# Kolkir/feature-point-cnn

Hardware: AMD Instinct MI355X
Metric: frames/sec (VGA 640x480) SuperPoint fwd+NMS+descriptors (higher is better)
Workload: dtype f32

## Files before the change

feature-point-cnn_amd/csrc/wblock36p_mfma.h:

```cpp
#pragma once
#include "wblock36_mfma.h"

namespace fpc {

template <int TYT_, int TXT_, bool DUST_ = false, bool CONV_ = false>
struct W36PCfg {
  static constexpr int TYT = TYT_, TXT = TXT_;
  static constexpr bool DUST = DUST_, CONV = CONV_;
  static_assert(TYT * TXT == 16 && (TYT == 4 || TYT == 2 || (CONV && !DUST && TYT == 8)), "16 Winograd tiles per workgroup tile: 4 x 4 or 2 x 8 (conv-only: or 8 x 2)");
  static constexpr int NT = 512, NTH = 256, NPOS = 36, KC = 16, N = 64;
  static constexpr int TH = 4 * TYT, TW = 4 * TXT, HH = TH + 2, HW = TW + 2, NHALO = HH * HW;
  static constexpr int HROW = 20;
  static constexpr int HIT = (NHALO * 5 + NTH - 1) / NTH;
  static constexpr int HALO_FLOATS = HIT * NTH * 4;
  static constexpr int V_FLOATS = NPOS * 16 * 16;
  static constexpr int OFF_V0 = 0, OFF_H1 = V_FLOATS, OFF_H0 = OFF_H1 + HALO_FLOATS, OFF_V1 = OFF_H0 + HALO_FLOATS;
  static constexpr int RH = N + 8;
  static constexpr int PX = TH * TW;
  static constexpr int T_FLOATS = PX * RH;
  static constexpr int BASE_FLOATS = (OFF_V1 + V_FLOATS) > (OFF_H0 + T_FLOATS) ? (OFF_V1 + V_FLOATS) : (OFF_H0 + T_FLOATS);
  static constexpr int HIT64 = (NHALO + NTH - 1) / NTH;
  static constexpr int D_HEAD = BASE_FLOATS, D_COL = D_HEAD + 64, D_UIN = D_HEAD + 448, D_V64 = D_UIN + 2304, D_M64 = D_V64 + 576, D_H64 = D_M64 + 576;
  static constexpr int LDS_FLOATS = DUST ? D_H64 + HIT64 * NTH * 4 : BASE_FLOATS;
  static constexpr int LDS_BYTES = LDS_FLOATS * 4;
  static_assert(LDS_BYTES <= 160 * 1024, "LDS");
  static constexpr int STEPS = 9;
  static constexpr int WPAD = W36Cfg<1, 4, 4>::WPAD, WPAD2 = W36Cfg<1, 4, 4>::WPAD2;
  static_assert(WPAD >= 36, "a wave prefetches up to one chunk past its stream's end");
};

template <int TYT, int TXT, int RING, bool DUST, bool CONV = false>
__device__ __forceinline__ void wblock36p_body(const WBlockArgs& a) {
  using C = W36PCfg<TYT, TXT, DUST, CONV>;
  constexpr int TH = C::TH, TW = C::TW, HW = C::HW, HH = C::HH, HROW = C::HROW, HIT = C::HIT, NTH = C::NTH;
  constexpr int N = C::N, RH = C::RH, STEPS = C::STEPS, PX = C::PX;
  static_assert(STEPS % RING == 0 && RING >= 2, "ring slots must line up across chunks");
  extern __shared__ __attribute__((aligned(16))) float lds[];
  f32x4* const lds4 = reinterpret_cast<f32x4*>(lds);
  constexpr int TL4 = C::OFF_H0 / 4;

  const int tid = threadIdx.x, lane = tid & 63;
  const unsigned lane16 = (unsigned)lane * 16u;
  const int wave = __builtin_amdgcn_readfirstlane(tid >> 6);
  const int grp = wave & 3;
  const int hs = wave >> 2;
  const int tiles = a.tiles_x * a.tiles_y;
  const int nchunk = a.nchunk;
  const float4* const w1h = a.w1 + (size_t)blockIdx.y * (a.ysplit_floats / 4);
  const float* const b1h = a.b1 + (size_t)blockIdx.y * a.ysplit_floats;

  const bool xcd_order = a.xcd_order && (gridDim.x & 7) == 0;
  const int wg_step = xcd_order ? (int)(gridDim.x >> 3) : (int)gridDim.x;
  const int xchunk = (a.total + 7) >> 3;
  const int wg_first = xcd_order ? (int)(blockIdx.x & 7) * xchunk + (int)(blockIdx.x >> 3) : (int)blockIdx.x;
  const int wg_end = xcd_order ? min(a.total, ((int)(blockIdx.x & 7) + 1) * xchunk) : a.total;
  if (wg_first >= wg_end) return;

  const __amdgpu_buffer_rsrc_t xrsrc = __builtin_amdgcn_make_buffer_rsrc(const_cast<float*>(a.x), 0, (int)a.x_bytes, 0x00020000);
  struct TilePos { int b, ty, tx, live; };
  auto tile_pos = [&](int wg) {
    TilePos q;
    q.live = wg < wg_end;
    const int wgc = q.live ? wg : wg_first;
    const int bl = wgc / tiles;
    const int t = wgc - bl * tiles;
    q.b = a.frame0 + bl;
    q.ty = t / a.tiles_x;
    q.tx = t - q.ty * a.tiles_x;
    return q;
  };
  auto halo_base = [&](const TilePos& q) {
    return __builtin_amdgcn_readfirstlane(((q.b * a.H + q.ty * TH) * a.W + q.tx * TW) * a.csx * 4);
  };
  constexpr bool KEEP_HYX = !DUST;
  auto slot_hyx = [&](int tl, int i) {
    const int e = tl + i * NTH;
    const int pix = (e * 13108) >> 16, c4 = e - pix * 5;
    const int hy = HW == 18 ? (pix * 3641) >> 16 : HW == 34 ? (pix * 1928) >> 16 : (pix * 6554) >> 16;
    static_assert(HW == 18 || HW == 34 || HW == 10, "a division constant per halo width");
    const int hx = pix - hy * HW;
    const bool slot_ok = (hy < HH) & (c4 < 4);
    return slot_ok ? (hy << 16) | (c4 << 8) | hx : 0x7fff0000;
  };
  int okoff[HIT];
  [[maybe_unused]] int hyx[KEEP_HYX ? HIT : 1];
  if (hs == 1) {
    const int tl = tid & (NTH - 1);
#pragma unroll
    for (int i = 0; i < HIT; ++i) {
      if constexpr (KEEP_HYX) hyx[i] = slot_hyx(tl, i);
      okoff[i] = W36_MARKER;
    }
  }
  [[maybe_unused]] int okoff64[C::HIT64];
  auto slot_hyx64 = [&](int tl, int i) {
    const int pix = tl + i * NTH;
    const int hy = HW == 18 ? (pix * 3641) >> 16 : HW == 34 ? (pix * 1928) >> 16 : (pix * 6554) >> 16;
    const int hx = pix - hy * HW;
    return (hy < HH && a.dust_in) ? (hy << 16) | hx : 0x7fff0000;
  };
  if constexpr (DUST) {
    if (hs == 1) {
#pragma unroll
      for (int i = 0; i < C::HIT64; ++i) okoff64[i] = W36_MARKER;
    }
  }
  auto halo_tile = [&](const TilePos& q) {
    const int iy0 = q.ty * TH - 1, ix0 = q.tx * TW - 1;
    const int hlim = q.live ? a.H : 0;
    int tlq = tid & (NTH - 1);
    asm volatile("" : "+v"(tlq));
#pragma unroll
    for (int i = 0; i < HIT; ++i) {
      int hv = KEEP_HYX ? hyx[KEEP_HYX ? i : 0] : slot_hyx(tlq, i);
      asm volatile("" : "+v"(hv));
      const int hy = hv >> 16, hx = hv & 0xff, c4 = (hv >> 8) & 0xff;
      const bool ok = ((unsigned)(iy0 + hy) < (unsigned)hlim) & ((unsigned)(ix0 + hx) < (unsigned)a.W);
      okoff[i] = ok ? (((hy - 1) * a.W + (hx - 1)) * a.csx + c4 * 4) * 4 : W36_MARKER;
    }
    if constexpr (DUST) {
#pragma unroll
      for (int i = 0; i < C::HIT64; ++i) {
        int hv = slot_hyx64(tlq, i);
        asm volatile("" : "+v"(hv));
        const int hy = hv >> 16, hx = hv & 0xffff;
        const bool ok = ((unsigned)(iy0 + hy) < (unsigned)hlim) & ((unsigned)(ix0 + hx) < (unsigned)a.W);
        okoff64[i] = ok ? (((hy - 1) * a.W + (hx - 1)) * a.csx + 64) * 4 : W36_MARKER;
      }
    }
  };
  auto load_halo64 = [&](int base) {
    if constexpr (DUST) {
#pragma unroll
      for (int i = 0; i < C::HIT64; ++i) {
        int voff;
        asm("v_add_i32 %0, %1, %2 clamp" : "=v"(voff) : "v"(okoff64[i]), "s"(base));
        __builtin_amdgcn_raw_ptr_buffer_load_lds(xrsrc, (__attribute__((address_space(3))) void*)(lds + C::D_H64 + (i * NTH + grp * 64) * 4), 16, voff, 0, 0, 0);
      }
    }
  };
  auto load_halo = [&](int base, int hoff_f) {
#pragma unroll
    for (int i = 0; i < HIT; ++i) {
      int voff;
      asm("v_add_i32 %0, %1, %2 clamp" : "=v"(voff) : "v"(okoff[i]), "s"(base));
      __builtin_amdgcn_raw_ptr_buffer_load_lds(xrsrc, (__attribute__((address_space(3))) void*)(lds + hoff_f + (i * NTH + grp * 64) * 4), 16, voff, 0, 0, 0);
    }
  };
  const int tq = tid & (NTH - 1);
  const int wt_t = tq >> 4, ch_t = tq & 15;
  const int m_t = ((wt_t & 7) >> 1) * 4 + (wt_t >> 3) * 2 + (wt_t & 1);
  const int trd = ((4 * (wt_t / TXT)) * HW + 4 * (wt_t % TXT)) * HROW + ch_t;
  const int twr = m_t * 16 + ((((ch_t >> 2) ^ (2 * ((m_t >> 3) & 1))) << 2) | (ch_t & 3));
  typedef float f32x2 __attribute__((ext_vector_type(2)));
  f32x2 tp[6][3];
  auto t_read = [&](int rd, int i, int j) { tp[i][j >> 1][j & 1] = lds[rd + (i * HW + j) * HROW]; };
  auto bt6 = [&](f32x2& x0, f32x2& x1, f32x2& x2, f32x2& x3, f32x2& x4, f32x2& x5) {
    const f32x2 k4 = {4.f, 4.f}, km4 = {-4.f, -4.f}, k5 = {-5.f, -5.f}, k2 = {2.f, 2.f}, km2 = {-2.f, -2.f};
    const f32x2 p = __builtin_elementwise_fma(km4, x2, x4), q = __builtin_elementwise_fma(km4, x1, x3);
    const f32x2 r = x4 - x2, s = x3 - x1;
    const f32x2 y0 = __builtin_elementwise_fma(k4, x0, __builtin_elementwise_fma(k5, x2, x4));
    const f32x2 y5 = __builtin_elementwise_fma(k4, x1, __builtin_elementwise_fma(k5, x3, x5));
    x0 = y0;
    x1 = p + q;
    x2 = p - q;
    x3 = __builtin_elementwise_fma(k2, s, r);
    x4 = __builtin_elementwise_fma(km2, s, r);
    x5 = y5;
  };
  auto t_burst = [&]() {
#pragma unroll
    for (int jj = 0; jj < 3; ++jj) bt6(tp[0][jj], tp[1][jj], tp[2][jj], tp[3][jj], tp[4][jj], tp[5][jj]);
#pragma unroll
    for (int ii = 0; ii < 3; ++ii)
#pragma unroll
      for (int jj = 0; jj < 3; ++jj) {
        const f32x2 ra = tp[2 * ii][jj], rb = tp[2 * ii + 1][jj];
        tp[2 * ii][jj] = __builtin_shufflevector(ra, rb, 0, 2);
        tp[2 * ii + 1][jj] = __builtin_shufflevector(ra, rb, 1, 3);
      }
#pragma unroll
    for (int ii = 0; ii < 3; ++ii) bt6(tp[2 * ii][0], tp[2 * ii + 1][0], tp[2 * ii][1], tp[2 * ii + 1][1], tp[2 * ii][2], tp[2 * ii + 1][2]);
  };
  auto t_write = [&](int wr, int i, int j) { lds[wr + (i * 6 + j) * 256] = tp[2 * (i >> 1) + (j & 1)][j >> 1][i & 1]; };

  const int aoff4 = (lane & 15) * 4 + ((lane >> 4) ^ (2 * ((lane & 15) >> 3))) + hs * 18 * 64;
  const unsigned gstride = ((unsigned)nchunk * 36u + (unsigned)C::WPAD) * 1024u;
  const __amdgpu_buffer_rsrc_t wrsrc = __builtin_amdgcn_make_buffer_rsrc(const_cast<float4*>(w1h), 0, (int)(4u * gstride), 0x00020000);
  const unsigned wlane = (unsigned)grp * gstride + (unsigned)hs * (18u * 1024u) + lane16;
  struct BF { f32x4 v[2]; };
  auto ldb = [&](int cc, int s) {
    BF r;
#pragma unroll
    for (int q = 0; q < 2; ++q)
      r.v[q] = __builtin_bit_cast(f32x4, __builtin_amdgcn_raw_buffer_load_b128(wrsrc, (int)wlane, cc * (36 * 1024) + (2 * s + q) * 1024, 0));
    return r;
  };

  [[maybe_unused]] int d_va = 0, d_ua = 0;
  [[maybe_unused]] const __amdgpu_buffer_rsrc_t drsrc =
      DUST ? __builtin_amdgcn_make_buffer_rsrc(const_cast<float*>(a.dust + W36Dust::UOUT), 0, nchunk * 36 * 16 * 4, 0x00020000) : xrsrc;
  [[maybe_unused]] f32x4 du[6];
  [[maybe_unused]] float dacc[9];
  if constexpr (DUST) {
    d_va = grp * 64 + lane;
    d_ua = grp * 64 + 16 * ((lane & 3) ^ (2 * (lane >> 5)));
    for (int i = tid; i < 448 / 4; i += C::NT) lds4[C::D_HEAD / 4 + i] = reinterpret_cast<const f32x4*>(a.dust)[i];
    for (int i = tid; i < 2304 / 4; i += C::NT) lds4[C::D_UIN / 4 + i] = reinterpret_cast<const f32x4*>(a.dust + W36Dust::UIN)[i];
  }

  TilePos pos_cur = tile_pos(wg_first);
  int base_cur = halo_base(pos_cur);
  if (hs == 1) {
    halo_tile(pos_cur);
    load_halo64(base_cur);
    load_halo(base_cur, C::OFF_H0);
    load_halo(base_cur + 64, C::OFF_H1);
    asm volatile("s_waitcnt vmcnt(%0)" ::"n"(HIT) : "memory");
  }
  FPC_LDS_BARRIER();
  if (hs == 0) {
#pragma unroll
    for (int i = 0; i < 6; ++i)
#pragma unroll
      for (int j = 0; j < 6; ++j) t_read(trd + C::OFF_H0, i, j);
    t_burst();
#pragma unroll
    for (int i = 0; i < 6; ++i)
#pragma unroll
      for (int j = 0; j < 6; ++j) t_write(twr + C::OFF_V0, i, j);
  }
  FPC_LDS_BARRIER();

  constexpr int C4 = N / 4, EIT = PX * C4 / C::NT, PPI = C::NT / C4;
  constexpr int RPI = PPI / TW > 0 ? PPI / TW : 1;
  const __amdgpu_buffer_rsrc_t orsrc = __builtin_amdgcn_make_buffer_rsrc(a.out + blockIdx.y * N, 0, W36_MARKER, 0x00020000);
  const int g2s = __builtin_amdgcn_readfirstlane(((a.k8_h + a.k8_x) / 2 + C::WPAD2) * 64);
  const __amdgpu_buffer_rsrc_t w2rsrc = __builtin_amdgcn_make_buffer_rsrc(const_cast<float4*>(a.w2), 0, a.conv_only ? 0 : 4 * g2s * 16, 0x00020000);
  const unsigned w2lane = (unsigned)(grp * g2s) * 16u + lane16;

  const int wg_stamp = wg_first + 2 * wg_step < wg_end ? wg_first + 2 * wg_step : wg_first;
  for (int wg = wg_first; wg < wg_end; wg += wg_step) {
    const int b = pos_cur.b, ty = pos_cur.ty, tx = pos_cur.tx;
    const TilePos pos_next = tile_pos(wg + wg_step);
    const int base_next = halo_base(pos_next);
    if (wg == wg_stamp) { FPC_STAMP(0) FPC_RSTAMP(6) }

    f32x4 acc[18];
    {
      float zf = 0.f;
      asm volatile("" : "+v"(zf));
#pragma unroll
      for (int p = 0; p < 18; ++p) acc[p] = f32x4{zf, zf, zf, zf};
    }
    if constexpr (DUST) {
      float zf = 0.f;
      asm volatile("" : "+v"(zf));
#pragma unroll
      for (int i = 0; i < 9; ++i) dacc[i] = zf;
    }
    BF bq[RING];
#pragma unroll
    for (int i = 0; i < RING - 1; ++i) bq[i] = ldb(0, i);

    auto chunk_body = [&](auto ROLE, auto PAR, const int c) {
      constexpr int role = decltype(ROLE)::value, par = decltype(PAR)::value;
      constexpr int VB_OFF = par ? C::OFF_V1 : C::OFF_V0, VN_OFF = par ? C::OFF_V0 : C::OFF_V1;
      constexpr int HS_OFF = par ? C::OFF_H1 : C::OFF_H0;
      constexpr int HN_OFF = par ? C::OFF_H0 : C::OFF_H1;
      const int c3 = c + 2;
      const bool nxt = c3 >= nchunk;
      const int l_base = (nxt ? base_next : base_cur) + (nxt ? c3 - nchunk : c3) * 64;
      int ao = aoff4 + VB_OFF / 4, trd_c = trd + HN_OFF, twr_c = twr + VN_OFF;
      asm volatile("" : "+v"(ao), "+v"(trd_c), "+v"(twr_c));
      [[maybe_unused]] int dva = d_va + VB_OFF / 4;
      [[maybe_unused]] f32x4 dv[3];
      if constexpr (DUST) asm volatile("" : "+v"(dva));
      f32x4 ac[2][2];
#pragma unroll
      for (int q = 0; q < 2; ++q) ac[0][q] = lds4[ao + q * 64];
      fpc_static_for<STEPS>([&](auto S) __attribute__((always_inline)) {
        constexpr int s = decltype(S)::value;
        {
          constexpr int t = s + RING - 1;
          if constexpr (t < STEPS) bq[t % RING] = ldb(c, t);
          else bq[t % RING] = ldb(c + 1, t - STEPS);
        }
        if (s + 1 < STEPS) {
#pragma unroll
          for (int q = 0; q < 2; ++q) ac[(s + 1) & 1][q] = lds4[ao + ((s + 1) * 2 + q) * 64];
        }
        constexpr int SPS = 4;
#pragma unroll
        for (int u = 0; u < SPS; ++u) {
          const int slot = s * SPS + u;
          if constexpr (role == 1) {
            if (slot == 1) {
              if (c3 == nchunk) halo_tile(pos_next);
              load_halo(l_base, HS_OFF);
            }
            if constexpr (DUST) {
              auto dread = [&](int i0) {
#pragma unroll
                for (int k = 0; k < 3; ++k) dv[k] = lds4[dva + (i0 + k) * 256];
              };
              auto dfma = [&](int i0) {
#pragma unroll
                for (int k = 0; k < 3; ++k)
#pragma unroll
                  for (int e = 0; e < 4; ++e) dacc[i0 + k] = __builtin_fmaf(dv[k][e], du[(i0 / 3 % 2) * 3 + k][e], dacc[i0 + k]);
              };
              auto dload = [&](int i0) {
#pragma unroll
                for (int k = 0; k < 3; ++k)
                  du[(i0 / 3 % 2) * 3 + k] = __builtin_bit_cast(f32x4, __builtin_amdgcn_raw_buffer_load_b128(drsrc, d_ua + (i0 + k) * 256, c * (36 * 16 * 4), 0));
              };
              if (slot == 3) dload(0);
              else if (slot == 11) dread(0);
              else if (slot == 13) { dfma(0); dload(3); }
              else if (slot == 21) dread(3);
              else if (slot == 23) { dfma(3); dload(6); }
              else if (slot == 31) dread(6);
              else if (slot == 33) dfma(6);
            }
          } else {
            if (slot >= 2 && slot < 14) {
#pragma unroll
              for (int k = 0; k < 3; ++k) { const int e = (slot - 2) * 3 + k; t_read(trd_c, e / 6, e % 6); }
            } else if (slot == 14) {
              t_burst();
            } else if (slot >= 15 && slot < 33) {
#pragma unroll
              for (int k = 0; k < 2; ++k) { const int e = (slot - 15) * 2 + k; t_write(twr_c, e / 6, e % 6); }
            }
          }
        }
        __builtin_amdgcn_sched_barrier(0);
        fpc_mfma_step<false, false>(acc[2 * s], acc[2 * s + 1], ac[s & 1][0], ac[s & 1][1], bq[s % RING].v[0], bq[s % RING].v[1]);
        __builtin_amdgcn_sched_barrier(0);
      });
      asm volatile("s_waitcnt vmcnt(%0)" ::"n"(2 * (STEPS - 1)) : "memory");
      FPC_LDS_BARRIER();
    };
    __builtin_amdgcn_s_waitcnt(0x0F70);
    if (hs == 0) {
      int c = 0;
      do {
        chunk_body(std::integral_constant<int, 0>{}, std::integral_constant<int, 0>{}, c);
        chunk_body(std::integral_constant<int, 0>{}, std::integral_constant<int, 1>{}, c + 1);
        c += 2;
      } while (c < nchunk);
    } else {
      int c = 0;
      do {
        chunk_body(std::integral_constant<int, 1>{}, std::integral_constant<int, 0>{}, c);
        chunk_body(std::integral_constant<int, 1>{}, std::integral_constant<int, 1>{}, c + 1);
        c += 2;
      } while (c < nchunk);
    }
    if (wg == wg_stamp) { FPC_STAMP(1) }
    asm volatile("s_nop 15\n\ts_nop 7" ::: "memory");

    int tid_t = tid;
    asm volatile("" : "+v"(tid_t));
    const int lane_t = tid_t & 63, n16 = lane_t & 15, kq = lane_t >> 4;
    const bool proj = a.k8_x > 0;
    if constexpr (DUST) {
      if (a.dust_in) {
        if (tid_t < 16) {
          const int rd = C::D_H64 + ((4 * (tid_t / TXT)) * HW + 4 * (tid_t % TXT)) * 4;
#pragma unroll
          for (int i = 0; i < 6; ++i)
#pragma unroll
            for (int j = 0; j < 6; ++j) tp[i][j >> 1][j & 1] = lds[rd + (i * HW + j) * 4];
          t_burst();
          const int mrow = ((tid_t & 7) >> 1) * 4 + (tid_t >> 3) * 2 + (tid_t & 1);
#pragma unroll
          for (int i = 0; i < 6; ++i)
#pragma unroll
            for (int j = 0; j < 6; ++j) lds[C::D_V64 + (i * 6 + j) * 16 + mrow] = tp[2 * (i >> 1) + (j & 1)][j >> 1][i & 1];
        }
        FPC_LDS_BARRIER();
        {
          const int va = C::D_V64 + hs * 18 * 16 + (lane_t & 15), ub = C::D_UIN + grp * 576 + hs * 18 * 16 + (lane_t & 15);
          float av[18], bv[18];
#pragma unroll
          for (int p = 0; p < 18; ++p) {
            av[p] = lds[va + p * 16];
            bv[p] = lds[ub + p * 16];
          }
          __builtin_amdgcn_sched_barrier(0);
#pragma unroll
          for (int p = 0; p < 18; ++p) {
            const float x = lane_t < 16 ? av[p] : 0.f;
            acc[p] = __builtin_amdgcn_mfma_f32_16x16x4f32(x, bv[p], acc[p], 0, 0, 0);
          }
        }
      }
      if (hs == 1) {
        const int m_d = lane_t >> 2;
#pragma unroll
        for (int i = 0; i < 9; ++i) {
          float v = dacc[i];
          v += __shfl_xor(v, 1);
          v += __shfl_xor(v, 2);
          const int pos = grp + 4 * i;
          if (a.dust_in) v = __builtin_fmaf(lds[C::D_V64 + pos * 16 + m_d], lds[C::D_HEAD + W36Dust::UIN64 + pos], v);
          if ((lane_t & 3) == 0) lds[C::D_M64 + pos * 16 + m_d] = v;
        }
      }
      FPC_LDS_BARRIER();
      if (hs == 1) load_halo64(base_next);
    }

    int hw_base[4];
#pragma unroll
    for (int r = 0; r < 4; ++r) {
      const int T = 8 * (r >> 1) + 2 * kq + (r & 1);
      hw_base[r] = C::OFF_H0 + ((4 * (T / TXT)) * TW + 4 * (T % TXT)) * RH + 16 * grp + n16;
    }
    auto out_transform = [&](auto ROLE) __attribute__((always_inline)) {
      constexpr int role = decltype(ROLE)::value;
      auto partial = [&](int rp, f32x2 (&yv)[4][4]) {
        f32x2 tt[4][6];
#pragma unroll
        for (int j = 0; j < 6; ++j) {
          auto pr = [&](int pos) { return f32x2{acc[pos][2 * rp], acc[pos][2 * rp + 1]}; };
          const f32x2 ma = pr(0 * 6 + j), mb = pr(1 * 6 + j), mc = pr(2 * 6 + j);
          if constexpr (role == 0) {
            const f32x2 s12 = mb + mc, d12 = mb - mc;
            tt[0][j] = ma + s12;
            tt[1][j] = d12;
            tt[2][j] = s12;
            tt[3][j] = d12;
          } else {
            const f32x2 s34 = ma + mb, d34 = ma - mb;
            tt[0][j] = s34;
            tt[1][j] = f32x2{2.f, 2.f} * d34;
            tt[2][j] = f32x2{4.f, 4.f} * s34;
            tt[3][j] = __builtin_elementwise_fma(f32x2{8.f, 8.f}, d34, mc);
          }
        }
#pragma unroll
        for (int i = 0; i < 4; ++i) {
          const f32x2 m0 = tt[i][0], m1 = tt[i][1], m2 = tt[i][2], m3 = tt[i][3], m4 = tt[i][4], m5 = tt[i][5];
          const f32x2 s12 = m1 + m2, d12 = m1 - m2, s34 = m3 + m4, d34 = m3 - m4;
          yv[i][0] = m0 + s12 + s34;
          yv[i][1] = __builtin_elementwise_fma(f32x2{2.f, 2.f}, d34, d12);
          yv[i][2] = __builtin_elementwise_fma(f32x2{4.f, 4.f}, s34, s12);
          yv[i][3] = __builtin_elementwise_fma(f32x2{8.f, 8.f}, d34, d12) + m5;
        }
      };
      {
        f32x2 yv[4][4];
        partial(1 - role, yv);
#pragma unroll
        for (int e = 0; e < 2; ++e)
#pragma unroll
          for (int i = 0; i < 4; ++i) lds4[TL4 + (e * 4 + i) * C::NT + tid_t] = f32x4{yv[i][0][e], yv[i][1][e], yv[i][2][e], yv[i][3][e]};
      }
      FPC_LDS_BARRIER();
      {
        f32x4 other[2][4];
#pragma unroll
        for (int e = 0; e < 2; ++e)
#pragma unroll
          for (int i = 0; i < 4; ++i) other[e][i] = lds4[TL4 + (e * 4 + i) * C::NT + (tid_t ^ NTH)];
        f32x2 yv[4][4];
        partial(role, yv);
        const float bias1 = b1h[16 * grp + n16];
        float hv[2][16];
#pragma unroll
        for (int i = 0; i < 4; ++i)
#pragma unroll
          for (int jj = 0; jj < 4; ++jj)
#pragma unroll
            for (int e = 0; e < 2; ++e) {
              const float v = (yv[i][jj][e] + other[e][i][jj]) + bias1;
              hv[e][i * 4 + jj] = v > 0.f ? v : 0.f;
            }
        FPC_LDS_BARRIER();
#pragma unroll
        for (int e = 0; e < 2; ++e)
#pragma unroll
          for (int i = 0; i < 4; ++i)
#pragma unroll
            for (int jj = 0; jj < 4; ++jj) lds[hw_base[2 * role + e] + (i * TW + jj) * RH] = hv[e][i * 4 + jj];
        if constexpr (DUST && role == 0) {
          if (tid_t < 16) {
            float mm[36];
#pragma unroll
            for (int p = 0; p < 36; ++p) mm[p] = lds[C::D_M64 + p * 16 + tid_t];
            const float bias64 = lds[C::D_HEAD + W36Dust::B1];
            float tt[4][6];
#pragma unroll
            for (int j = 0; j < 6; ++j) {
              const float m0 = mm[0 * 6 + j], m1 = mm[1 * 6 + j], m2 = mm[2 * 6 + j], m3 = mm[3 * 6 + j], m4 = mm[4 * 6 + j], m5 = mm[5 * 6 + j];
              const float s12 = m1 + m2, d12 = m1 - m2, s34 = m3 + m4, d34 = m3 - m4;
              tt[0][j] = m0 + s12 + s34;
              tt[1][j] = __builtin_fmaf(2.f, d34, d12);
              tt[2][j] = __builtin_fmaf(4.f, s34, s12);
              tt[3][j] = __builtin_fmaf(8.f, d34, d12) + m5;
            }
            const int T = 8 * ((tid_t >> 1) & 1) + 2 * (tid_t >> 2) + (tid_t & 1);
            const int hb = C::OFF_H0 + ((4 * (T / TXT)) * TW + 4 * (T % TXT)) * RH + 64;
#pragma unroll
            for (int i = 0; i < 4; ++i) {
              const float m0 = tt[i][0], m1 = tt[i][1], m2 = tt[i][2], m3 = tt[i][3], m4 = tt[i][4], m5 = tt[i][5];
              const float s12 = m1 + m2, d12 = m1 - m2, s34 = m3 + m4, d34 = m3 - m4;
              float yv64[4];
              yv64[0] = m0 + s12 + s34 + bias64;
              yv64[1] = __builtin_fmaf(2.f, d34, d12) + bias64;
              yv64[2] = __builtin_fmaf(4.f, s34, s12) + bias64;
              yv64[3] = __builtin_fmaf(8.f, d34, d12) + m5 + bias64;
#pragma unroll
              for (int jj = 0; jj < 4; ++jj) lds[hb + (i * TW + jj) * RH] = yv64[jj] > 0.f ? yv64[jj] : 0.f;
            }
          }
        }
      }
      FPC_LDS_BARRIER();
    };
    if (hs == 0) out_transform(std::integral_constant<int, 0>{});
    else out_transform(std::integral_constant<int, 1>{});
    if (wg == wg_stamp) { FPC_STAMP(2) }

    const int y0 = ty * TH, x0 = tx * TW;
    const int rows_valid = min(TH, a.H - y0);
    const int xbase = __builtin_amdgcn_readfirstlane(((b * a.H + y0) * a.W + x0) * a.csx * 4);
    const int obase = __builtin_amdgcn_readfirstlane(((b * a.H + y0) * a.W + x0) * a.cso * 4);
    const int m0 = tid_t / C4, c4t = tid_t - m0 * C4;
    const int rsub = __builtin_amdgcn_readfirstlane(m0 / TW), pcol = m0 % TW;
    const int ocol = (x0 + pcol < a.W) ? (pcol * a.cso + c4t * 4) * 4 : W36_MARKER;
    int erd = TL4 + m0 * (RH / 4) + c4t;
    asm volatile("" : "+v"(erd));
    auto store_out = [&]() {
#pragma unroll
      for (int i = 0; i < EIT; ++i) {
        const int prow = i * RPI + rsub;
        if (prow < rows_valid) {
          f32x4 v = lds4[erd + i * PPI * (RH / 4)];
          if (!CONV && !a.conv_only) {
            v.x = v.x > 0.f ? v.x : 0.f;
            v.y = v.y > 0.f ? v.y : 0.f;
            v.z = v.z > 0.f ? v.z : 0.f;
            v.w = v.w > 0.f ? v.w : 0.f;
          }
          int voff;
          const int so = obase + prow * a.W * a.cso * 4;
          asm("v_add_i32 %0, %1, %2 clamp" : "=v"(voff) : "v"(ocol), "s"(so));
          __builtin_amdgcn_raw_buffer_store_b128(__builtin_bit_cast(__attribute__((__vector_size__(4 * sizeof(unsigned)))) unsigned, v), orsrc, voff, 0, 0);
        }
      }
    };

    if (CONV || a.conv_only) {
      store_out();
      FPC_LDS_BARRIER();
    } else if constexpr (!CONV) {
      f32x4 acc2[8];
      const int pb = hs;
      [[maybe_unused]] float dpart[8];
      [[maybe_unused]] float dw2r = 0.f;
      [[maybe_unused]] float dhv[8][4];
      [[maybe_unused]] const int dq = lane_t & 15, dpxl = lane_t >> 4;
      [[maybe_unused]] float dx64 = 0.f;
      if constexpr (DUST) {
        if (!proj) {
          const int px = 32 * wave + 4 * (dq >> 1) + dpxl;
          dx64 = __builtin_bit_cast(float, __builtin_amdgcn_raw_buffer_load_b32(xrsrc, (((px / TW) * a.W + px % TW) * a.csx + 64) * 4, xbase, 0));
        }
        const f32x4 wq = lds4[C::D_COL / 4 + dq];
        const float w64 = dq == 0 ? lds[C::D_COL + 64] : 0.f;
#pragma unroll
        for (int it = 0; it < 8; ++it) {
          const int px = 32 * wave + 4 * it + dpxl;
          const f32x4 hq = lds4[TL4 + px * (RH / 4) + dq];
          const float h64 = lds[C::OFF_H0 + px * RH + 64];
          float v = h64 * w64;
#pragma unroll
          for (int e = 0; e < 4; ++e) v = __builtin_fmaf(hq[e], wq[e], v);
          dpart[it] = v;
        }
        dw2r = lds[C::D_HEAD + W36Dust::W2ROW + 16 * grp + n16];
#pragma unroll
        for (int mb = 0; mb < 8; ++mb)
#pragma unroll
          for (int r = 0; r < 4; ++r) dhv[mb][r] = lds[C::OFF_H0 + (128 * pb + 16 * mb + 4 * kq + r) * RH + 64];
      }
      auto ldb2 = [&](int s) {
        return __builtin_bit_cast(f32x4, __builtin_amdgcn_raw_buffer_load_b128(w2rsrc, (int)w2lane, s * 1024, 0));
      };
      constexpr int KH = N / 16;
      auto gemm_over = [&](int ksteps, int s_first) {
        int ar = TL4 + (128 * pb + n16) * (RH / 4) + kq;
        asm volatile("" : "+v"(ar));
        f32x4 cb[4];
#pragma unroll
        for (int i = 0; i < 3; ++i) cb[i] = ldb2(s_first + i);
        f32x4 af[2][2];
#pragma unroll
        for (int q = 0; q < 2; ++q) af[0][q] = lds4[ar + q * 16 * (RH / 4)];
        for (int g = 0; g < ksteps; g += 4) {
#pragma unroll
          for (int u = 0; u < 4; ++u) {
            cb[(u + 3) & 3] = ldb2(s_first + g + u + 3);
            fpc_static_for<4>([&](auto B_) __attribute__((always_inline)) {
              constexpr int blk = decltype(B_)::value;
              if (blk + 1 < 4) {
#pragma unroll
                for (int q = 0; q < 2; ++q) af[(blk + 1) & 1][q] = lds4[ar + (g + u) * 4 + ((blk + 1) * 2 + q) * 16 * (RH / 4)];
              } else {
#pragma unroll
                for (int q = 0; q < 2; ++q) af[(blk + 1) & 1][q] = lds4[ar + (g + u + 1) * 4 + q * 16 * (RH / 4)];
              }
              __builtin_amdgcn_sched_barrier(0);
              fpc_mfma_step<false, false>(acc2[2 * blk], acc2[2 * blk + 1], af[blk & 1][0], af[blk & 1][1], cb[u], cb[u]);
              __builtin_amdgcn_sched_barrier(0);
            });
          }
        }
      };
      if (proj) {
        constexpr int XIT = PX * 16 / C::NT;
        f32x4 xst[XIT];
        auto load_x = [&](int pass) {
          const int kx4 = min(16, a.k8_x * 2 - pass * 16);
          const int px0 = tid_t >> 4;
          const int xp = (((px0 / TW) * a.W + px0 % TW) * a.csx + ((tid_t & 15) < kx4 ? pass * 64 + (tid_t & 15) * 4 : 0)) * 4;
#pragma unroll
          for (int i = 0; i < XIT; ++i) {
            const int so = xbase + i * RPI * a.W * a.csx * 4;
            xst[i] = __builtin_bit_cast(f32x4, __builtin_amdgcn_raw_buffer_load_b128(xrsrc, xp + so, 0, 0));
          }
        };
        load_x(0);
        {
          float zf = 0.f;
          asm volatile("" : "+v"(zf));
#pragma unroll
          for (int mb = 0; mb < 8; ++mb) acc2[mb] = f32x4{zf, zf, zf, zf};
          if constexpr (DUST) {
#pragma unroll
            for (int mb = 0; mb < 8; ++mb)
#pragma unroll
              for (int r = 0; r < 4; ++r) acc2[mb][r] = dhv[mb][r] * dw2r;
          }
        }
        gemm_over(KH, 0);
        if (wg == wg_stamp) { FPC_STAMP(3) }
        const int npass = (a.k8_x + 7) >> 3;
        for (int pass = 0; pass < npass; ++pass) {
          FPC_LDS_BARRIER();
          {
            int xw = TL4 + (tid_t >> 4) * (RH / 4) + (tid_t & 15);
            asm volatile("" : "+v"(xw));
#pragma unroll
            for (int i = 0; i < XIT; ++i) lds4[xw + i * 32 * (RH / 4)] = xst[i];
          }
          FPC_LDS_BARRIER();
          if (pass + 1 < npass) load_x(pass + 1);
          if constexpr (DUST) {
            const f32x4 wa = lds4[C::D_COL / 4 + 20 + pass * 16 + dq];
#pragma unroll
            for (int it = 0; it < 8; ++it) {
              const int px = 32 * wave + 4 * it + dpxl;
              const f32x4 xa = lds4[TL4 + px * (RH / 4) + dq];
              float v = dpart[it];
#pragma unroll
              for (int e = 0; e < 4; ++e) v = __builtin_fmaf(xa[e], wa[e], v);
              dpart[it] = v;
            }
          }
          const int steps = min(4, a.k8_x / 2 - pass * 4);
          gemm_over(steps, KH + pass * 4);
        }
      } else {
        int xl = (4 * kq * a.csx + 16 * grp + n16) * 4;
        asm volatile("" : "+v"(xl));
#pragma unroll
        for (int mb = 0; mb < 8; ++mb)
#pragma unroll
          for (int r = 0; r < 4; ++r) {
            constexpr int BPR = TW / 16;
            const int mbg = 8 * pb + mb;
            const int so = xbase + ((mbg / BPR) * a.W + (mbg % BPR) * 16 + r) * a.csx * 4;
            acc2[mb][r] = __builtin_bit_cast(float, __builtin_amdgcn_raw_buffer_load_b32(xrsrc, xl, so, 0));
          }
        if constexpr (DUST) {
#pragma unroll
          for (int mb = 0; mb < 8; ++mb)
#pragma unroll
            for (int r = 0; r < 4; ++r) acc2[mb][r] = __builtin_fmaf(dhv[mb][r], dw2r, acc2[mb][r]);
        }
        gemm_over(KH, 0);
        if (wg == wg_stamp) { FPC_STAMP(3) }
      }

      if (wg == wg_stamp) { FPC_STAMP(4) }
      asm volatile("s_nop 15\n\ts_nop 7" ::: "memory");
      FPC_LDS_BARRIER();
      {
        int ew = C::OFF_H0 + (128 * pb + 4 * kq) * RH + 16 * grp + n16;
        asm volatile("" : "+v"(ew));
        const float bias = a.b2[16 * grp + n16];
#pragma unroll
        for (int mb = 0; mb < 8; ++mb)
#pragma unroll
          for (int r = 0; r < 4; ++r) lds[ew + (16 * mb + r) * RH] = acc2[mb][r] + bias;
      }
      FPC_LDS_BARRIER();
      store_out();
      if constexpr (DUST) {
        const bool b3 = (dq & 8) != 0, b2 = (dq & 4) != 0, b1 = (dq & 2) != 0;
        float r1[4], r2[2];
#pragma unroll
        for (int k = 0; k < 4; ++k) r1[k] = (b3 ? dpart[4 + k] : dpart[k]) + __shfl_xor(b3 ? dpart[k] : dpart[4 + k], 8);
#pragma unroll
        for (int k = 0; k < 2; ++k) r2[k] = (b2 ? r1[2 + k] : r1[k]) + __shfl_xor(b2 ? r1[k] : r1[2 + k], 4);
        float tot = (b1 ? r2[1] : r2[0]) + __shfl_xor(b1 ? r2[0] : r2[1], 2);
        tot += __shfl_xor(tot, 1);
        const int dpx = 32 * wave + 4 * (dq >> 1) + dpxl, dhf = dq & 1, drow = dpx / TW, dcol = dpx % TW;
        tot += dx64 + lds[C::D_HEAD + W36Dust::B2];
        tot = tot > 0.f ? tot : 0.f;
        const bool ok = (drow < rows_valid) & (x0 + dcol < a.W);
        const int doff = ok ? ((drow * a.W + dcol) * a.cso + 64 + 4 * dhf) * 4 : W36_MARKER;
        int voff;
        asm("v_add_i32 %0, %1, %2 clamp" : "=v"(voff) : "v"(doff), "s"(obase));
        const f32x4 v = {dhf ? 0.f : tot, 0.f, 0.f, 0.f};
        __builtin_amdgcn_raw_buffer_store_b128(__builtin_bit_cast(__attribute__((__vector_size__(4 * sizeof(unsigned)))) unsigned, v), orsrc, voff, 0, 0);
      }
      if (wg == wg_stamp) { FPC_STAMP(5) FPC_RSTAMP(7) }
      FPC_LDS_BARRIER();
    }
    pos_cur = pos_next;
    base_cur = base_next;
  }
}

template <int TYT, int TXT, int RING = 3>
__global__ __launch_bounds__(512, 1) void wblock36p_kernel(const WBlockArgs a) {
  wblock36p_body<TYT, TXT, RING, false>(a);
}

template <int TYT, int TXT, int RING = 3>
__global__ __launch_bounds__(512, 1) void wconv36p_kernel(const WBlockArgs a) {
  wblock36p_body<TYT, TXT, RING, false, true>(a);
}

template <int TYT, int TXT, int RING = 3>
__global__ __launch_bounds__(512, 1) void wblock36p_dust_kernel(const WBlockArgs a) {
  wblock36p_body<TYT, TXT, RING, true>(a);
}

}
```

Baseline: 12380.

## Restructure dust-channel halo setup, 64th-channel output transform, and identity-load addressing

Splits the 64th-channel halo offset computation into its own lambda that runs per tile. It also keeps the precomputed halo coordinates in the dust variant too. The output transform for channel 64 is spread across four wave groups, one output row each, instead of running on 16 threads of role 0. Inline-asm v_fmac replaces the builtin fma in the dust accumulation, and the identity-add load addresses are built incrementally from scalar strides. The aim is to cut VALU and scalar address arithmetic and to balance the serial dust tail, at the cost of more live registers and redundant LDS reads of m-values per row.

```diff
diff --git a/feature-point-cnn_amd/csrc/wblock36p_mfma.h b/feature-point-cnn_amd/csrc/wblock36p_mfma.h
--- a/feature-point-cnn_amd/csrc/wblock36p_mfma.h
+++ b/feature-point-cnn_amd/csrc/wblock36p_mfma.h
@@ -29,6 +29,10 @@
   static_assert(WPAD >= 36, "a wave prefetches up to one chunk past its stream's end");
 };
 
+__device__ __forceinline__ void w36p_fmac(float& d, float x, float y) {
+  asm volatile("v_fmac_f32 %0, %1, %2" : "+v"(d) : "v"(x), "v"(y));
+}
+
 template <int TYT, int TXT, int RING, bool DUST, bool CONV = false>
 __device__ __forceinline__ void wblock36p_body(const WBlockArgs& a) {
   using C = W36PCfg<TYT, TXT, DUST, CONV>;
@@ -72,7 +76,6 @@
   auto halo_base = [&](const TilePos& q) {
     return __builtin_amdgcn_readfirstlane(((q.b * a.H + q.ty * TH) * a.W + q.tx * TW) * a.csx * 4);
   };
-  constexpr bool KEEP_HYX = !DUST;
   auto slot_hyx = [&](int tl, int i) {
     const int e = tl + i * NTH;
     const int pix = (e * 13108) >> 16, c4 = e - pix * 5;
@@ -83,12 +86,12 @@
     return slot_ok ? (hy << 16) | (c4 << 8) | hx : 0x7fff0000;
   };
   int okoff[HIT];
-  [[maybe_unused]] int hyx[KEEP_HYX ? HIT : 1];
+  int hyx[HIT];
   if (hs == 1) {
     const int tl = tid & (NTH - 1);
 #pragma unroll
     for (int i = 0; i < HIT; ++i) {
-      if constexpr (KEEP_HYX) hyx[i] = slot_hyx(tl, i);
+      hyx[i] = slot_hyx(tl, i);
       okoff[i] = W36_MARKER;
     }
   }
@@ -108,17 +111,21 @@
   auto halo_tile = [&](const TilePos& q) {
     const int iy0 = q.ty * TH - 1, ix0 = q.tx * TW - 1;
     const int hlim = q.live ? a.H : 0;
-    int tlq = tid & (NTH - 1);
-    asm volatile("" : "+v"(tlq));
 #pragma unroll
     for (int i = 0; i < HIT; ++i) {
-      int hv = KEEP_HYX ? hyx[KEEP_HYX ? i : 0] : slot_hyx(tlq, i);
+      int hv = hyx[i];
       asm volatile("" : "+v"(hv));
       const int hy = hv >> 16, hx = hv & 0xff, c4 = (hv >> 8) & 0xff;
       const bool ok = ((unsigned)(iy0 + hy) < (unsigned)hlim) & ((unsigned)(ix0 + hx) < (unsigned)a.W);
       okoff[i] = ok ? (((hy - 1) * a.W + (hx - 1)) * a.csx + c4 * 4) * 4 : W36_MARKER;
     }
+  };
+  auto halo_tile64 = [&](const TilePos& q) {
     if constexpr (DUST) {
+      const int iy0 = q.ty * TH - 1, ix0 = q.tx * TW - 1;
+      const int hlim = q.live ? a.H : 0;
+      int tlq = tid & (NTH - 1);
+      asm volatile("" : "+v"(tlq));
 #pragma unroll
       for (int i = 0; i < C::HIT64; ++i) {
         int hv = slot_hyx64(tlq, i);
@@ -203,7 +210,7 @@
   [[maybe_unused]] f32x4 du[6];
   [[maybe_unused]] float dacc[9];
   if constexpr (DUST) {
-    d_va = grp * 64 + lane;
+    d_va = grp * 64 + lane - aoff4;
     d_ua = grp * 64 + 16 * ((lane & 3) ^ (2 * (lane >> 5)));
     for (int i = tid; i < 448 / 4; i += C::NT) lds4[C::D_HEAD / 4 + i] = reinterpret_cast<const f32x4*>(a.dust)[i];
     for (int i = tid; i < 2304 / 4; i += C::NT) lds4[C::D_UIN / 4 + i] = reinterpret_cast<const f32x4*>(a.dust + W36Dust::UIN)[i];
@@ -213,6 +220,7 @@
   int base_cur = halo_base(pos_cur);
   if (hs == 1) {
     halo_tile(pos_cur);
+    halo_tile64(pos_cur);
     load_halo64(base_cur);
     load_halo(base_cur, C::OFF_H0);
     load_halo(base_cur + 64, C::OFF_H1);
@@ -273,9 +281,8 @@
       const int l_base = (nxt ? base_next : base_cur) + (nxt ? c3 - nchunk : c3) * 64;
       int ao = aoff4 + VB_OFF / 4, trd_c = trd + HN_OFF, twr_c = twr + VN_OFF;
       asm volatile("" : "+v"(ao), "+v"(trd_c), "+v"(twr_c));
-      [[maybe_unused]] int dva = d_va + VB_OFF / 4;
+      [[maybe_unused]] const int dva = ao + d_va;
       [[maybe_unused]] f32x4 dv[3];
-      if constexpr (DUST) asm volatile("" : "+v"(dva));
       f32x4 ac[2][2];
 #pragma unroll
       for (int q = 0; q < 2; ++q) ac[0][q] = lds4[ao + q * 64];
@@ -308,7 +315,8 @@
 #pragma unroll
                 for (int k = 0; k < 3; ++k)
 #pragma unroll
-                  for (int e = 0; e < 4; ++e) dacc[i0 + k] = __builtin_fmaf(dv[k][e], du[(i0 / 3 % 2) * 3 + k][e], dacc[i0 + k]);
+                  for (int e = 0; e < 4; ++e)
+                    w36p_fmac(dacc[i0 + k], dv[k][e], du[(i0 / 3 % 2) * 3 + k][e]);
               };
               auto dload = [&](int i0) {
 #pragma unroll
@@ -410,7 +418,10 @@
         }
       }
       FPC_LDS_BARRIER();
-      if (hs == 1) load_halo64(base_next);
+      if (hs == 1) {
+        halo_tile64(pos_next);
+        load_halo64(base_next);
+      }
     }
 
     int hw_base[4];
@@ -486,36 +497,41 @@
           for (int i = 0; i < 4; ++i)
 #pragma unroll
             for (int jj = 0; jj < 4; ++jj) lds[hw_base[2 * role + e] + (i * TW + jj) * RH] = hv[e][i * 4 + jj];
-        if constexpr (DUST && role == 0) {
-          if (tid_t < 16) {
-            float mm[36];
-#pragma unroll
-            for (int p = 0; p < 36; ++p) mm[p] = lds[C::D_M64 + p * 16 + tid_t];
+        if constexpr (DUST && role == 1) {
+          auto y64_row = [&](auto I_) __attribute__((always_inline)) {
+            constexpr int i = decltype(I_)::value;
+            int ma = C::D_M64 + lane_t;
+            asm volatile("" : "+v"(ma));
+            float tt[6];
+#pragma unroll
+            for (int j = 0; j < 6; ++j) {
+              auto mrd = [&](int r) { return lds[ma + (r * 6 + j) * 16]; };
+              const float m1 = mrd(1), m2 = mrd(2), m3 = mrd(3), m4 = mrd(4);
+              const float s12 = m1 + m2, d12 = m1 - m2, s34 = m3 + m4, d34 = m3 - m4;
+              if constexpr (i == 0) tt[j] = mrd(0) + s12 + s34;
+              else if constexpr (i == 1) tt[j] = __builtin_fmaf(2.f, d34, d12);
+              else if constexpr (i == 2) tt[j] = __builtin_fmaf(4.f, s34, s12);
+              else tt[j] = __builtin_fmaf(8.f, d34, d12) + mrd(5);
+            }
             const float bias64 = lds[C::D_HEAD + W36Dust::B1];
-            float tt[4][6];
-#pragma unroll
-            for (int j = 0; j < 6; ++j) {
-              const float m0 = mm[0 * 6 + j], m1 = mm[1 * 6 + j], m2 = mm[2 * 6 + j], m3 = mm[3 * 6 + j], m4 = mm[4 * 6 + j], m5 = mm[5 * 6 + j];
-              const float s12 = m1 + m2, d12 = m1 - m2, s34 = m3 + m4, d34 = m3 - m4;
-              tt[0][j] = m0 + s12 + s34;
-              tt[1][j] = __builtin_fmaf(2.f, d34, d12);
-              tt[2][j] = __builtin_fmaf(4.f, s34, s12);
-              tt[3][j] = __builtin_fmaf(8.f, d34, d12) + m5;
-            }
-            const int T = 8 * ((tid_t >> 1) & 1) + 2 * (tid_t >> 2) + (tid_t & 1);
-            const int hb = C::OFF_H0 + ((4 * (T / TXT)) * TW + 4 * (T % TXT)) * RH + 64;
-#pragma unroll
-            for (int i = 0; i < 4; ++i) {
-              const float m0 = tt[i][0], m1 = tt[i][1], m2 = tt[i][2], m3 = tt[i][3], m4 = tt[i][4], m5 = tt[i][5];
-              const float s12 = m1 + m2, d12 = m1 - m2, s34 = m3 + m4, d34 = m3 - m4;
-              float yv64[4];
-              yv64[0] = m0 + s12 + s34 + bias64;
-              yv64[1] = __builtin_fmaf(2.f, d34, d12) + bias64;
-              yv64[2] = __builtin_fmaf(4.f, s34, s12) + bias64;
-              yv64[3] = __builtin_fmaf(8.f, d34, d12) + m5 + bias64;
-#pragma unroll
-              for (int jj = 0; jj < 4; ++jj) lds[hb + (i * TW + jj) * RH] = yv64[jj] > 0.f ? yv64[jj] : 0.f;
-            }
+            const int T = 8 * ((lane_t >> 1) & 1) + 2 * (lane_t >> 2) + (lane_t & 1);
+            int hb = C::OFF_H0 + ((4 * (T / TXT)) * TW + 4 * (T % TXT)) * RH + 64;
+            asm volatile("" : "+v"(hb));
+            const float m0 = tt[0], m1 = tt[1], m2 = tt[2], m3 = tt[3], m4 = tt[4], m5 = tt[5];
+            const float s12 = m1 + m2, d12 = m1 - m2, s34 = m3 + m4, d34 = m3 - m4;
+            float yv64[4];
+            yv64[0] = m0 + s12 + s34 + bias64;
+            yv64[1] = __builtin_fmaf(2.f, d34, d12) + bias64;
+            yv64[2] = __builtin_fmaf(4.f, s34, s12) + bias64;
+            yv64[3] = __builtin_fmaf(8.f, d34, d12) + m5 + bias64;
+#pragma unroll
+            for (int jj = 0; jj < 4; ++jj) lds[hb + (i * TW + jj) * RH] = yv64[jj] > 0.f ? yv64[jj] : 0.f;
+          };
+          if (lane_t < 16) {
+            if (grp == 0) y64_row(std::integral_constant<int, 0>{});
+            else if (grp == 1) y64_row(std::integral_constant<int, 1>{});
+            else if (grp == 2) y64_row(std::integral_constant<int, 2>{});
+            else y64_row(std::integral_constant<int, 3>{});
           }
         }
       }
@@ -560,6 +576,11 @@
     } else if constexpr (!CONV) {
       f32x4 acc2[8];
       const int pb = hs;
+      constexpr int BPR = TW / 16;
+      int px4 = a.csx * 4, row4 = a.W * a.csx * 4;
+      asm volatile("" : "+s"(px4), "+s"(row4));
+      int id_row0 = xbase + (8 / BPR) * pb * row4;
+      asm volatile("" : "+s"(id_row0));
       [[maybe_unused]] float dpart[8];
       [[maybe_unused]] float dw2r = 0.f;
       [[maybe_unused]] float dhv[8][4];
@@ -678,15 +699,17 @@
       } else {
         int xl = (4 * kq * a.csx + 16 * grp + n16) * 4;
         asm volatile("" : "+v"(xl));
-#pragma unroll
-        for (int mb = 0; mb < 8; ++mb)
+        int so_row = id_row0;
+#pragma unroll
+        for (int mb = 0; mb < 8; ++mb) {
+          if (mb > 0 && mb % BPR == 0) so_row += row4;
+          int so = so_row + (mb % BPR) * 16 * px4;
 #pragma unroll
           for (int r = 0; r < 4; ++r) {
-            constexpr int BPR = TW / 16;
-            const int mbg = 8 * pb + mb;
-            const int so = xbase + ((mbg / BPR) * a.W + (mbg % BPR) * 16 + r) * a.csx * 4;
             acc2[mb][r] = __builtin_bit_cast(float, __builtin_amdgcn_raw_buffer_load_b32(xrsrc, xl, so, 0));
-          }
+            so += px4;
+          }
+        }
         if constexpr (DUST) {
 #pragma unroll
           for (int mb = 0; mb < 8; ++mb)
```

New measurement: 12420, median of 6. No clear change (+0.3%).
